# 0xC0000054/avif-format

Hardware: AMD Instinct MI355X
Metric: Mpixels/s + achieved HBM GB/s, 8K 32bpc→10-bit Rec.2100 PQ, 1 GPU (higher is better)
Workload: dtype f32

## Files before the change

avif-format_amd/csrc/device_math.h:

```cpp
#pragma once
#include <hip/hip_runtime.h>
#include <stdint.h>

namespace avifgpu {

#define AG_DEV __device__ __forceinline__

AG_DEV float nat_log2(float x) { return __builtin_amdgcn_logf(x); }
AG_DEV float nat_exp2(float x) { return __builtin_amdgcn_exp2f(x); }
AG_DEV float nat_rcp(float x)  { return __builtin_amdgcn_rcpf(x); }
AG_DEV float nat_sqrt(float x) { return __builtin_amdgcn_sqrtf(x); }

AG_DEV float max0(float v) { return __int_as_float(max(__float_as_int(v), 0)); }

AG_DEV float fast_pow(float x, float e) { return nat_exp2(e * nat_log2(x)); }

AG_DEV float fast_rcp_nr(float d)
{
    const float r = nat_rcp(d);
    return __builtin_fmaf(__builtin_fmaf(-d, r, 1.0f), r, r);
}

constexpr float kPqM1 = 2610.0f / 16384.0f;
constexpr float kPqM2 = 2523.0f / 4096.0f * 128.0f;
// ... 32 lines not shown
    const f32x2 l = { nat_log2(value.x), nat_log2(value.y) };
#endif
    const f32x2 e1 = __builtin_elementwise_fma((f32x2)kPqM1, l, (f32x2)log2_mult_m1);
    const f32x2 x = { nat_exp2(e1.x), nat_exp2(e1.y) };
    const f32x2 n = kPqC1 + kPqC2 * x;
    const f32x2 d = 1.0f + kPqC3 * x;
    const f32x2 r = { nat_rcp(d.x), nat_rcp(d.y) };
    const f32x2 q0 = n * r;
    const f32x2 q = __builtin_elementwise_fma(__builtin_elementwise_fma(-q0, d, n), r, q0);
    const f32x2 e2 = kPqM2 * f32x2{ nat_log2(q.x), nat_log2(q.y) };
    return f32x2{ nat_exp2_sat(e2.x), nat_exp2_sat(e2.y) };
}
AG_DEV float fast_linear_to_pq(float value, float mult)
{
    return fast_linear_to_pq01(value, kPqM1 * nat_log2(mult));
}

#ifndef AG_PQ_TAB_FORM
#define AG_PQ_TAB_FORM 2
#endif
#ifndef AG_PQ_ND_FMA
#define AG_PQ_ND_FMA 0
#endif
constexpr int kPqTabEntries = 512;
constexpr int kPqTabPad = 4;
constexpr int kPqTabCount = AG_PQ_TAB_FORM == 3 ? 3 : 2;
struct PqExpTable { float t[kPqTabCount][kPqTabEntries + kPqTabPad]; };
constexpr int kPqTabFloats = kPqTabCount * (kPqTabEntries + kPqTabPad);
constexpr float pq_pow2(int n) { float v = 1.0f; for (int i = 0; i < (n < 0 ? -n : n); ++i) v = n < 0 ? v * 0.5f : v * 2.0f; return v; }
constexpr PqExpTable make_pq_exp_table()
{
    PqExpTable t{};
    for (int i = 0; i < kPqTabEntries; ++i) {
        const int eb = i & 255;
        float F = 0.0f;
        int N = -100;
        if (i < 256 && eb != 0 && eb != 255) {
            const long long num = 2610LL * (eb - 126);
            long long n = (num + 8192) >> 14;
            if (((num + 8192) & 16383) == 0 && (n & 1)) n -= 1;
            F = (float)(num - n * 16384) / 16384.0f;
            N = (int)n;
        }
        if (AG_PQ_TAB_FORM == 3) { t.t[0][i] = F; t.t[1][i] = kPqC2 * pq_pow2(N); t.t[kPqTabCount - 1][i] = kPqC3 * pq_pow2(N); }
        else if (AG_PQ_TAB_FORM == 2) { t.t[0][i] = F; t.t[1][i] = pq_pow2(N); }
        else { constexpr int W = kPqTabEntries + kPqTabPad; t.t[(2 * i) / W][(2 * i) % W] = F; t.t[(2 * i + 1) / W][(2 * i + 1) % W] = pq_pow2(N); }
    }
    return t;
}
__device__ __attribute__((aligned(16))) const PqExpTable kPqExpTableConst = make_pq_exp_table();
static_assert(sizeof(PqExpTable) == kPqTabFloats * sizeof(float) && kPqTabFloats % 4 == 0, "copied as float4");
AG_DEV float* pq_exp_table()
{
    __shared__ __attribute__((aligned(16))) float tab[kPqTabFloats];
    return tab;
}
AG_DEV void pq_exp_table_fill(int tid, int nthreads)
{
    typedef float f4 __attribute__((ext_vector_type(4)));
    f4* dst = reinterpret_cast<f4*>(pq_exp_table());
    const f4* src = reinterpret_cast<const f4*>(&kPqExpTableConst);
    for (int i = tid; i < kPqTabFloats / 4; i += nthreads) dst[i] = src[i];
}
template <int NTHREADS> struct PqTableFill {
    typedef float f4 __attribute__((ext_vector_type(4)));
    static constexpr int kVec = kPqTabFloats / 4, N = (kVec + NTHREADS - 1) / NTHREADS;
    f4 v[N];
    AG_DEV void load(int tid)
    {
        const f4* src = reinterpret_cast<const f4*>(&kPqExpTableConst);
#pragma unroll
        for (int i = 0; i < N; ++i) { const int idx = tid + i * NTHREADS; v[i] = src[idx < kVec ? idx : kVec - 1]; }
        __builtin_amdgcn_sched_barrier(0);
    }
    AG_DEV void store(int tid)
    {
        f4* dst = reinterpret_cast<f4*>(pq_exp_table());
#pragma unroll
        for (int i = 0; i < N; ++i) { const int idx = tid + i * NTHREADS; dst[idx < kVec ? idx : kVec - 1] = v[i]; }
    }
};
AG_DEV void pq_table_barrier()
{
    __builtin_amdgcn_fence(__ATOMIC_RELEASE, "workgroup", "local");
    __builtin_amdgcn_s_barrier();
    __builtin_amdgcn_fence(__ATOMIC_ACQUIRE, "workgroup", "local");
}
AG_DEV uint32_t pq_tab_offset(float t) { return (__float_as_uint(t) >> (AG_PQ_TAB_FORM == 1 ? 20 : 21)) & (AG_PQ_TAB_FORM == 1 ? 0xff8u : 0x7fcu); }
AG_DEV float pq_tab_at(const float* tab, int which, uint32_t off)
{
    if (AG_PQ_TAB_FORM == 1) return *reinterpret_cast<const float*>(reinterpret_cast<const uint8_t*>(tab + which) + off);
    return *reinterpret_cast<const float*>(reinterpret_cast<const uint8_t*>(tab + which * (kPqTabEntries + kPqTabPad)) + off);
}
AG_DEV float pq_mantissa(float t) { return __uint_as_float((__float_as_uint(t) & 0x007fffffu) | 0x3f000000u); }
AG_DEV float fast_linear_to_pq01_hi(float value, float mult)
{
    const float* tab = pq_exp_table();
    const float t = value * mult;
    const uint32_t off = pq_tab_offset(t);
    const float y = nat_exp2(__builtin_fmaf(kPqM1, nat_log2(pq_mantissa(t)), pq_tab_at(tab, 0, off)));
    float n, d;
    if (AG_PQ_TAB_FORM == 3 && AG_PQ_ND_FMA) { n = __builtin_fmaf(pq_tab_at(tab, 1, off), y, kPqC1); d = __builtin_fmaf(pq_tab_at(tab, 2, off), y, 1.0f); }
    else if (AG_PQ_TAB_FORM == 3) { n = kPqC1 + pq_tab_at(tab, 1, off) * y; d = 1.0f + pq_tab_at(tab, 2, off) * y; }
    else if (AG_PQ_ND_FMA) { const float x = y * pq_tab_at(tab, 1, off); n = __builtin_fmaf(kPqC2, x, kPqC1); d = __builtin_fmaf(kPqC3, x, 1.0f); }
    else { const float x = y * pq_tab_at(tab, 1, off); n = kPqC1 + kPqC2 * x; d = 1.0f + kPqC3 * x; }
    return nat_exp2_sat(kPqM2 * nat_log2(near_ieee_div(n, d)));
}
AG_DEV f32x2 fast_linear_to_pq01_2_hi(f32x2 value, float mult)
{
    const float* tab = pq_exp_table();
    const f32x2 t = value * mult;
    const uint32_t o0 = pq_tab_offset(t.x), o1 = pq_tab_offset(t.y);
    const f32x2 F = { pq_tab_at(tab, 0, o0), pq_tab_at(tab, 0, o1) };
    const f32x2 l = { nat_log2(pq_mantissa(t.x)), nat_log2(pq_mantissa(t.y)) };
    const f32x2 e1 = __builtin_elementwise_fma((f32x2)kPqM1, l, F);
    const f32x2 y = { nat_exp2(e1.x), nat_exp2(e1.y) };
    f32x2 n, d;
// ... 403 lines not shown
```

avif-format_amd/csrc/write_kernels.hip:

```cpp
#include <hip/hip_runtime.h>
#include <cstdio>
#include <cstdlib>
#include <cstring>
#include <type_traits>
#include "kernel_params.h"
#include "staging.h"
#include "device_math.h"
#include "satword_f32.h"
#include "icc_pipeline32.h"
#include "../../include/avifgpu.h"

#pragma clang fp contract(off)

namespace avifgpu {

#ifndef AG_WRITE_PART
#define AG_WRITE_PART 0
#endif
constexpr bool kHerePlain  = AG_WRITE_PART != 36 && AG_WRITE_PART != 38 && AG_WRITE_PART != 1;
constexpr bool kHereIcc6   = AG_WRITE_PART == 0 || AG_WRITE_PART == 36;
constexpr bool kHereIcc8   = AG_WRITE_PART == 0 || AG_WRITE_PART == 38;
hipError_t launch_planes_d8(const WriteParams& p, int planes, bool dst16, int output, int xs, int ys, hipStream_t st, char* label);
hipError_t launch_planes_d16(const WriteParams& p, int planes, bool dst16, int output, int xs, int ys, hipStream_t st, char* label);
hipError_t launch_planes_d32(const WriteParams& p, int planes, bool dst16, int output, int xs, int ys, hipStream_t st, char* label);
// ... 1069 lines not shown
                        constexpr int v1 = YS ? 1 : 0;
                        R = (R + qflt(0, i0 + i1o, 0) + qflt(v1, i0, 0) + qflt(v1, i0 + i1o, 0)) * 0.25f;
                        G = (G + qflt(0, i0 + i1o, 1) + qflt(v1, i0, 1) + qflt(v1, i0 + i1o, 1)) * 0.25f;
                        B = (B + qflt(0, i0 + i1o, 2) + qflt(v1, i0, 2) + qflt(v1, i0 + i1o, 2)) * 0.25f;
                    }
                }
                const float cb = R * p.mcb[0] + G * p.mcb[1] + B * p.mcb[2];
                const float cr = R * p.mcr[0] + G * p.mcr[1] + B * p.mcr[2];
                cbv[j] = clip_round(cb + p.half, p.maxv);
                crv[j] = clip_round(cr + p.half, p.maxv);
            }
            const int ncvalid = (nvalid + (1 << XS) - 1) >> XS;
            store_samples<DST16, NC, true, ALIGNED>(p.dst[1] + (long long)gy * p.dst_stride[1] + (long long)(x0 >> XS) * DSZ, cbv, ncvalid);
            store_samples<DST16, NC, true, ALIGNED>(p.dst[2] + (long long)gy * p.dst_stride[2] + (long long)(x0 >> XS) * DSZ, crv, ncvalid);
        }
    }
}

#ifndef AG_STREAM_BLOCK
#define AG_STREAM_BLOCK 128
#endif
constexpr int kStreamWaves = AG_STREAM_BLOCK / 64;
#ifndef AG_F32_REF_BLOCK
#define AG_F32_REF_BLOCK 256
#endif
constexpr int kF32RefWaves = AG_F32_REF_BLOCK / 64;

typedef float    f32x4 __attribute__((ext_vector_type(4)));
typedef uint32_t u32x4 __attribute__((ext_vector_type(4)));
typedef uint32_t u32x2 __attribute__((ext_vector_type(2)));

typedef int i32x4 __attribute__((__vector_size__(16)));
typedef int i32x2 __attribute__((__vector_size__(8)));
AG_DEV __amdgpu_buffer_rsrc_t span_rsrc(const void* base, uint32_t bytes)
{
    return __builtin_amdgcn_make_buffer_rsrc(const_cast<void*>(base), 0, (int)bytes, 0x00020000);
}
template <bool NT> AG_DEV f32x4 span_load16(__amdgpu_buffer_rsrc_t r, uint32_t voff, uint32_t soff)
{
    if constexpr (AG_MATH_ONLY) return mo_value<f32x4>();
    const i32x4 v = __builtin_amdgcn_raw_buffer_load_b128(r, (int)voff, (int)soff, NT ? 2 : 0);
    return __builtin_bit_cast(f32x4, v);
}
template <bool NT> AG_DEV void span_store16(__amdgpu_buffer_rsrc_t r, uint32_t voff, u32x4 v)
{
    if constexpr (AG_MATH_ONLY) mo_sink(v); else __builtin_amdgcn_raw_buffer_store_b128(__builtin_bit_cast(i32x4, v), r, (int)voff, 0, NT ? 2 : 0);
}
template <bool NT> AG_DEV void span_store8(__amdgpu_buffer_rsrc_t r, uint32_t voff, u32x2 v)
// ... 136 lines not shown
#define AG_RGBA_PRIO 0
#endif
#ifndef AG_REF_PRIO
#define AG_REF_PRIO 0
#endif
#ifndef AG_INT_PRIO
#define AG_INT_PRIO 1
#endif
#ifndef AG_PREMUL_PAIR
#define AG_PREMUL_PAIR 1
#endif
#ifndef AG_REF_BUFFER_STORES
#define AG_REF_BUFFER_STORES 0
#endif
#ifndef AG_RGB16_BUFFER
#define AG_RGB16_BUFFER 0
#endif
#ifndef AG_IREF_BUFFER
#define AG_IREF_BUFFER 1
#endif
#ifndef AG_HOT444_BLOCK
#define AG_HOT444_BLOCK AG_F32_STREAM_BLOCK
#endif
#ifndef AG_MEASURE
#define AG_MEASURE 0
#endif
#ifndef AG_HOT444_GLOBAL
#define AG_HOT444_GLOBAL 0
#endif
constexpr int kHot444Waves = AG_HOT444_BLOCK / 64;
template <int TRANSFER, int PXL, bool NT>
__global__ __launch_bounds__(AG_HOT444_BLOCK) AG_F32_SGPRS void write_rgb32_ycbcr444_hot(const WriteParams p)
{
    constexpr int WPB = kHot444Waves;
    constexpr int K = 3 * PXL / 4;
    constexpr int SPAN_PX = 64 * PXL;
    constexpr int SPAN_DW = AG_HOT_F32_STRIP ? SpanStrip<K>::kDwords : SPAN_PX * 3 / 2;
    constexpr int LDW = 3 * PXL / 2;
    __shared__ __attribute__((aligned(16))) uint32_t strip[WPB][SPAN_DW];
    constexpr bool LATE = AG_PQ_LATE_FILL && TRANSFER == kTransferPqHi && !AG_HOT_PREFETCH;
    constexpr bool PRIO = AG_HOT_PRIO && TRANSFER == kTransferPqHi;
    if constexpr (PRIO) __builtin_amdgcn_s_setprio(3);
    PqTableFill<AG_HOT444_BLOCK> tfill;
    if constexpr (LATE) tfill.load((int)threadIdx.x); else pq_prologue<TRANSFER>();

    const int wave = wave_in_block();
    const int lane = threadIdx.x & 63;
    uint32_t* my = strip[wave];

    const uint32_t spans_per_row = ((uint32_t)p.width + SPAN_PX - 1) / SPAN_PX;
    const uint32_t total = spans_per_row * (uint32_t)p.nrows;
    const uint32_t step = gridDim.x * WPB;
    const uint32_t voff = (uint32_t)lane * 16u;

    auto issue = [&](uint32_t s, f32x4 (&dst)[K]) {
        const uint32_t r = s / spans_per_row;
        const uint32_t sx = s - r * spans_per_row;
        const int span_px = s < total ? min(SPAN_PX, p.width - (int)sx * SPAN_PX) : 0;
        if constexpr (AG_HOT444_GLOBAL && !AG_HOT_PREFETCH) {
            if (span_px == SPAN_PX) {
                const f32x4* g = reinterpret_cast<const f32x4*>(p.src + (long long)r * p.src_row_bytes + (long long)sx * (SPAN_PX * 12)) + lane;
#pragma unroll
                for (int k = 0; k < K; ++k) dst[k] = stream_load<NT>(g + 64 * k);
                return;
            }
        }
        const __amdgpu_buffer_rsrc_t rs = span_rsrc(p.src + (long long)(s < total ? r : 0) * p.src_row_bytes + (long long)(s < total ? sx : 0) * (SPAN_PX * 12), (uint32_t)span_px * 12u);
#pragma unroll
        for (int k = 0; k < K; ++k) dst[k] = span_load_cached(k, K) ? span_load16<false>(rs, voff, 1024u * k) : span_load16<NT>(rs, voff, 1024u * k);
    };
    f32x4 nxt[AG_HOT_PREFETCH ? K : 1];
    if constexpr (AG_HOT_PREFETCH) issue(blockIdx.x * WPB + wave, nxt);
    f32x4 cur[K];
    if constexpr (!AG_HOT_PREFETCH) issue(blockIdx.x * WPB + wave, cur);
    if constexpr (PRIO) __builtin_amdgcn_s_setprio(0);
    if constexpr (LATE) {
        tfill.store((int)threadIdx.x);
        pq_table_barrier();
    }
    for (uint32_t sidx = blockIdx.x * WPB + wave; sidx < total; sidx += step) {
        const uint32_t r = sidx / spans_per_row;
        const uint32_t sx = sidx - r * spans_per_row;
        const int span_px = min(SPAN_PX, p.width - (int)sx * SPAN_PX);
        if constexpr (AG_HOT_PREFETCH) {
#pragma unroll
            for (int k = 0; k < K; ++k) cur[k] = nxt[k];
            issue(sidx + step, nxt);
            __builtin_amdgcn_sched_barrier(0);
        }

        float R[PXL], G[PXL], B[PXL];
        if constexpr (AG_HOT_F32_STRIP) {
#pragma unroll
            for (int k = 0; k < K; ++k) cur[k] = oetf_level4<TRANSFER>(p, cur[k]);
            float c[3 * PXL];
            span_transpose<K>(reinterpret_cast<f32x4*>(my), lane, cur, c);
#pragma unroll
            for (int i = 0; i < PXL; ++i) { R[i] = c[strip_at(i, 0)]; G[i] = c[strip_at(i, 1)]; B[i] = c[strip_at(i, 2)]; }
        } else {
#pragma unroll
            for (int k = 0; k < K; ++k) {
// ... 86 lines not shown
    const IccPowTableF powT = { pow_t };
    const int wave = wave_in_block();
    const int lane = threadIdx.x & 63;
    const uint32_t voff = (uint32_t)lane * 16u;
    f32x4* my = reinterpret_cast<f32x4*>(strip[wave]);
    const float m0 = p.icc_m_f[0], m1 = p.icc_m_f[1], m2 = p.icc_m_f[2], m3 = p.icc_m_f[3], m4 = p.icc_m_f[4], m5 = p.icc_m_f[5],
                m6 = p.icc_m_f[6], m7 = p.icc_m_f[7], m8 = p.icc_m_f[8];
    const uint32_t spans_per_row = ((uint32_t)p.width + SPAN_PX - 1) / SPAN_PX;
    const uint32_t total = spans_per_row * (uint32_t)p.nrows;
    const uint32_t step = gridDim.x * kF32Waves;
    f32x4 cur[K];
    auto issue = [&](uint32_t s) {
        const uint32_t r = s / spans_per_row;
        const uint32_t sx = s - r * spans_per_row;
        const int span_px = s < total ? min(SPAN_PX, p.width - (int)sx * SPAN_PX) : 0;
        const __amdgpu_buffer_rsrc_t rs = span_rsrc(p.src + (long long)(s < total ? r : 0) * p.src_row_bytes + (long long)(s < total ? sx : 0) * (SPAN_PX * 12), (uint32_t)span_px * 12u);
#pragma unroll
        for (int k = 0; k < K; ++k) cur[k] = span_load_cached(k, K) ? span_load16<false>(rs, voff, 1024u * k) : span_load16<true>(rs, voff, 1024u * k);
    };
    issue(blockIdx.x * kF32Waves + wave);
    if constexpr (AG_SUB_PRIO && !OUTREF) __builtin_amdgcn_s_setprio(0);
    if constexpr (LATE) {
        tfill.store((int)threadIdx.x);
        pq_table_barrier();
    }
    for (uint32_t sidx = blockIdx.x * kF32Waves + wave; sidx < total; sidx += step) {
        const uint32_t r = sidx / spans_per_row;
        const uint32_t sx = sidx - r * spans_per_row;
        const int span_px = min(SPAN_PX, p.width - (int)sx * SPAN_PX);
        if constexpr (ICCV == 2) {
            const IccSimple q = icc_simple_load(p);
#pragma unroll
            for (int k = 0; k < K; ++k) icc_trc_simple4(q, cur[k]);
        }
        float c[PXL * 3];
        span_transpose<K>(my, lane, cur, c);
        uint32_t yv[PXL], cbv[PXL], crv[PXL];
        uint32_t pk[OUTREF ? 12 : 1];
#pragma unroll
        for (int i = 0; i < PXL; i += 2) {
            float t[6], q[6];
#pragma unroll
            for (int h = 0; h < 2; ++h) {
                const float R0 = c[strip_at(i + h, 0)], G0 = c[strip_at(i + h, 1)], B0 = c[strip_at(i + h, 2)];
                t[3 * h] = __builtin_fmaf(B0, m2, __builtin_fmaf(G0, m1, R0 * m0));
                t[3 * h + 1] = __builtin_fmaf(B0, m5, __builtin_fmaf(G0, m4, R0 * m3));
                t[3 * h + 2] = __builtin_fmaf(B0, m8, __builtin_fmaf(G0, m7, R0 * m6));
// ... 68 lines not shown
    const uint32_t spans_per_row = ((uint32_t)p.width + SPAN_PX - 1) / SPAN_PX;
    const uint32_t groups = ((uint32_t)p.nrows + VR - 1) >> YS;
    const uint32_t total = spans_per_row * groups;
    const uint32_t step = gridDim.x * kF32Waves;
    f32x4 v[VR][K];
    auto issue = [&](uint32_t s) {
        const uint32_t gy = s / spans_per_row;
        const uint32_t sx = s - gy * spans_per_row;
        const int span_px = s < total ? min(SPAN_PX, p.width - (int)sx * SPAN_PX) : 0;
#pragma unroll
        for (int vr = 0; vr < VR; ++vr) {
            const int r = s < total ? min((int)(gy * VR) + vr, p.rows_to_end - 1) : 0;
            const __amdgpu_buffer_rsrc_t rs = span_rsrc(p.src + (long long)r * p.src_row_bytes + (long long)(s < total ? sx : 0) * (SPAN_PX * 12), (uint32_t)span_px * 12u);
#pragma unroll
            for (int k = 0; k < K; ++k) v[vr][k] = span_load_cached(k, K) ? span_load16<false>(rs, voff, 1024u * k) : span_load16<true>(rs, voff, 1024u * k);
        }
    };
    const uint32_t w0 = blockIdx.x * kF32Waves + wave;
    auto span_of = [&](uint32_t it) -> uint32_t { return w0 + it * step; };
    issue(span_of(0));
    if constexpr (AG_SUB_PRIO) __builtin_amdgcn_s_setprio(0);
    if constexpr (LATE) {
        tfill.store((int)threadIdx.x);
        pq_table_barrier();
    }
    for (uint32_t it = 0, sidx = span_of(0); sidx < total; sidx = span_of(++it)) {
        const uint32_t gy = sidx / spans_per_row;
        const uint32_t sx = sidx - gy * spans_per_row;
        const int span_px = min(SPAN_PX, p.width - (int)sx * SPAN_PX);
        const int nv = span_px - PXL * lane;
        float acc[4][3];
#pragma unroll
        for (int vr = 0; vr < VR; ++vr) {
            float c[PXL * 3];
            if constexpr (ICC1) {
                if constexpr (ICCV == 2) {
                    const IccSimple q = icc_simple_load(p);
#pragma unroll
                    for (int k = 0; k < K; ++k) icc_trc_simple4(q, v[vr][k]);
                }
            } else {
#pragma unroll
                for (int k = 0; k < K; ++k) v[vr][k] = oetf_level4<TRANSFER>(p, v[vr][k]);
            }
            span_transpose<K>(reinterpret_cast<f32x4*>(my), lane, v[vr], c);
            if constexpr (ICC1) {
#pragma unroll
// ... 133 lines not shown
    constexpr int PXL = AG_RGBA_HOT_PXL, SPAN_PX = 64 * PXL;
    __shared__ __attribute__((aligned(16))) uint32_t strip[kRgbaWaves][SpanStrip<PXL>::kDwords];
    const int wave = wave_in_block();
    const int lane = threadIdx.x & 63;
    f32x4* my = reinterpret_cast<f32x4*>(strip[wave]);
    const uint32_t voff = (uint32_t)lane * 16u;

    const uint32_t spans_per_row = ((uint32_t)p.width + SPAN_PX - 1) / SPAN_PX;
    const uint32_t total = spans_per_row * (uint32_t)p.nrows;
    const uint32_t step = gridDim.x * kRgbaWaves;
    f32x4 v[PXL];
    auto issue = [&](uint32_t s) {
        const uint32_t r = s / spans_per_row;
        const uint32_t sx = s - r * spans_per_row;
        const int span_px = s < total ? min(SPAN_PX, p.width - (int)sx * SPAN_PX) : 0;
        const __amdgpu_buffer_rsrc_t rs = span_rsrc(p.src + (long long)(s < total ? r : 0) * p.src_row_bytes + (long long)(s < total ? sx : 0) * (SPAN_PX * 16), (uint32_t)span_px * 16u);
#pragma unroll
        for (int k = 0; k < PXL; ++k) v[k] = span_load16<true>(rs, voff, 1024u * k);
    };
    issue(blockIdx.x * kRgbaWaves + wave);
    if constexpr (AG_RGBA_PRIO) __builtin_amdgcn_s_setprio(0);
    if constexpr (LATE) {
        tfill.store((int)threadIdx.x);
        pq_table_barrier();
    }
    for (uint32_t sidx = blockIdx.x * kRgbaWaves + wave; sidx < total; sidx += step) {
        const uint32_t r = sidx / spans_per_row;
        const uint32_t sx = sidx - r * spans_per_row;
        const int span_px = min(SPAN_PX, p.width - (int)sx * SPAN_PX);
        rgba_levels<TRANSFER, ICCV, PXL>(p, v);
        float c[4 * PXL];
        span_transpose<PXL>(my, lane, v, c);
        f32x4 px[PXL];
#pragma unroll
        for (int j = 0; j < PXL; ++j) px[j] = f32x4{ c[4 * j], c[4 * j + 1], c[4 * j + 2], c[4 * j + 3] };
        uint32_t yv[PXL], cbv[PXL], crv[PXL], av[PXL];
#pragma unroll
        for (int i = 0; i < PXL; ++i) {
            const float R = px[i].x, G = px[i].y, B = px[i].z;
            av[i] = (uint32_t)px[i].w;
            yv[i] = luma_code_nc(p, R, G, B);
            cbv[i] = clip_round(R * p.mcb[0] + G * p.mcb[1] + B * p.mcb[2] + p.half, p.maxv);
            crv[i] = clip_round(R * p.mcr[0] + G * p.mcr[1] + B * p.mcr[2] + p.half, p.maxv);
        }
        const uint32_t* planes_v[4] = { yv, cbv, crv, av };
        const int nv = span_px - PXL * lane;
        const uint32_t svo = (uint32_t)lane * (PXL * 2u);
// ... 33 lines not shown
    f32x4* my = reinterpret_cast<f32x4*>(strip[wave]);
    const uint32_t voff = (uint32_t)lane * 16u;
    const uint32_t spans_per_row = ((uint32_t)p.width + SPAN_PX - 1) / SPAN_PX;
    const uint32_t groups = ((uint32_t)p.nrows + VR - 1) >> YS;
    const uint32_t total = spans_per_row * groups;
    const uint32_t step = gridDim.x * kRgbaWaves;
    f32x4 v[VR][PXL];
    auto issue = [&](uint32_t s) {
        const uint32_t gy = s / spans_per_row;
        const uint32_t sx = s - gy * spans_per_row;
        const int span_px = s < total ? min(SPAN_PX, p.width - (int)sx * SPAN_PX) : 0;
#pragma unroll
        for (int vr = 0; vr < VR; ++vr) {
            const int r = s < total ? min((int)(gy * VR) + vr, p.rows_to_end - 1) : 0;
            const __amdgpu_buffer_rsrc_t rs = span_rsrc(p.src + (long long)r * p.src_row_bytes + (long long)(s < total ? sx : 0) * (SPAN_PX * 16), (uint32_t)span_px * 16u);
#pragma unroll
            for (int k = 0; k < PXL; ++k) v[vr][k] = span_load16<true>(rs, voff, 1024u * k);
        }
    };
    issue(blockIdx.x * kRgbaWaves + wave);
    if constexpr (AG_RGBA_PRIO) __builtin_amdgcn_s_setprio(0);
    if constexpr (LATE) {
        tfill.store((int)threadIdx.x);
        pq_table_barrier();
    }
    for (uint32_t sidx = blockIdx.x * kRgbaWaves + wave; sidx < total; sidx += step) {
        const uint32_t gy = sidx / spans_per_row;
        const uint32_t sx = sidx - gy * spans_per_row;
        const int span_px = min(SPAN_PX, p.width - (int)sx * SPAN_PX);
        const int nv = span_px - PXL * lane;
        float acc[2][3];
#pragma unroll
        for (int vr = 0; vr < VR; ++vr) {
            rgba_levels<TRANSFER, 0, PXL>(p, v[vr]);
            float c[4 * PXL];
            span_transpose<PXL>(my, lane, v[vr], c);
            const int r = (int)(gy * VR) + vr;
            if (r < p.nrows) {
                uint32_t yv[PXL], av[PXL];
#pragma unroll
                for (int i = 0; i < PXL; ++i) { yv[i] = luma_code_nc(p, c[4 * i], c[4 * i + 1], c[4 * i + 2]); av[i] = (uint32_t)c[4 * i + 3]; }
                const long long xo = (long long)sx * (SPAN_PX * 2);
                span_store_samples4<true>(p.dst[0] + (long long)r * p.dst_stride[0] + xo, (uint32_t)span_px, (uint32_t)lane, u32x2{ yv[0] | (yv[1] << 16), yv[2] | (yv[3] << 16) });
                span_store_samples4<true>(p.dst[3] + (long long)r * p.dst_stride[3] + xo, (uint32_t)span_px, (uint32_t)lane, u32x2{ av[0] | (av[1] << 16), av[2] | (av[3] << 16) });
            }
            if constexpr (!NEAREST) {
                if (span_px & 1) {
// ... 817 lines not shown
    if constexpr (AG_REF_PRIO) __builtin_amdgcn_s_setprio(3);
    PqTableFill<AG_F32_REF_BLOCK> tfill;
    if constexpr (LATE) tfill.load((int)threadIdx.x); else pq_prologue<TRANSFER>();
    constexpr int K = 4;
    const int lane = threadIdx.x & 63;
    const int wave = wave_in_block();
    const uint32_t n4 = (uint32_t)p.width * PLANES / 4;
    const uint32_t chunks = (n4 + 64 * K - 1) / (64 * K);
    const uint32_t total = chunks * (uint32_t)p.nrows;
    const uint32_t step = gridDim.x * kF32RefWaves;
    f32x4 v[K];
    auto issue = [&](uint32_t w) {
        const uint32_t r = w / chunks;
        const uint32_t c = w - r * chunks;
        const __amdgpu_buffer_rsrc_t rs = span_rsrc(p.src + (long long)(w < total ? r : 0) * p.src_row_bytes, w < total ? n4 * 16u : 0u);
        const uint32_t vo = (c * (64 * K) + (uint32_t)lane) * 16u;
#pragma unroll
        for (int k = 0; k < K; ++k) v[k] = span_load16<true>(rs, vo, 1024u * k);
    };
    issue(blockIdx.x * kF32RefWaves + wave);
    if constexpr (AG_REF_PRIO) __builtin_amdgcn_s_setprio(0);
    if constexpr (LATE) {
        tfill.store((int)threadIdx.x);
        pq_table_barrier();
    }
    for (uint32_t widx = blockIdx.x * kF32RefWaves + wave; widx < total; widx += step) {
        const uint32_t r = widx / chunks;
        const uint32_t c = widx - r * chunks;
        u32x2* dp = reinterpret_cast<u32x2*>(p.dst[0] + (long long)r * p.dst_stride[0]);
        uint32_t idx[K];
#pragma unroll
        for (int k = 0; k < K; ++k) idx[k] = c * (64 * K) + 64 * k + lane;
#pragma unroll
        for (int k = 0; k < K; k += 2) {
            float t[8];
            uint32_t q[8], ca[2] = { 0, 0 };
#pragma unroll
            for (int h = 0; h < 2; ++h) {
                float s0 = v[k + h].x, s1 = v[k + h].y, s2 = v[k + h].z, s3 = v[k + h].w;
                if constexpr (PLANES == 4) {
                    const float a = cxx_clamp(s3, 0.0f, 1.0f);
                    if (p.premultiply && a < 1.0f) {
                        s0 = (a == 0.0f) ? 0.0f : cxx_clamp(s0, 0.0f, 1.0f) * a;
                        s1 = (a == 0.0f) ? 0.0f : cxx_clamp(s1, 0.0f, 1.0f) * a;
                        s2 = (a == 0.0f) ? 0.0f : cxx_clamp(s2, 0.0f, 1.0f) * a;
                    }
                    ca[h] = (uint32_t)__builtin_amdgcn_fmed3f(a * p.maxf, 0.0f, p.maxf);
// ... 7 lines not shown
                const float tc[6] = { t[0], t[1], t[2], t[4], t[5], t[6] };
                uint32_t qc[6];
                oetf_codes<TRANSFER>(p, tc, qc);
                q[0] = qc[0]; q[1] = qc[1]; q[2] = qc[2]; q[3] = ca[0]; q[4] = qc[3]; q[5] = qc[4]; q[6] = qc[5]; q[7] = ca[1];
            } else {
                oetf_codes<TRANSFER>(p, t, q);
            }
#pragma unroll
            for (int h = 0; h < 2; ++h) {
                u32x2 o = { q[4 * h] | (q[4 * h + 1] << 16), q[4 * h + 2] | (q[4 * h + 3] << 16) };
                if constexpr (AG_REF_BUFFER_STORES) {
                    span_store8<true>(span_rsrc(dp, n4 * 8u), idx[k + h] * 8u, o);
                } else {
                    if (idx[k + h] >= n4) continue;
                    stream_store<true>(dp + idx[k + h], o);
                }
            }
        }
        if (widx + step < total) issue(widx + step);
    }
}

template <int DEPTH, int TRANSFER>
__global__ __launch_bounds__(AG_F32_REF_BLOCK) void write_ga_stream(const WriteParams p)
{
    static_assert(DEPTH == 16 || DEPTH == 32, "u16 or f32 samples");
    constexpr bool LATE = AG_PQ_LATE_FILL && DEPTH == 32 && TRANSFER == kTransferPqHi;
    PqTableFill<AG_F32_REF_BLOCK> tfill;
    if constexpr (LATE) tfill.load((int)threadIdx.x); else if constexpr (DEPTH == 32) pq_prologue<TRANSFER>();
    constexpr int K = 4;
    constexpr int PXV = DEPTH == 16 ? 4 : 2;
    const int lane = threadIdx.x & 63;
    const int wave = wave_in_block();
    const uint32_t nv = (uint32_t)p.width / PXV;
    const uint32_t chunks = (nv + 64 * K - 1) / (64 * K);
    const uint32_t total = chunks * (uint32_t)p.nrows;
    const uint32_t step = gridDim.x * kF32RefWaves;
    f32x4 v[K];
    auto issue = [&](uint32_t w) {
        const uint32_t r = w / chunks;
        const uint32_t c = w - r * chunks;
        const __amdgpu_buffer_rsrc_t rs = span_rsrc(p.src + (long long)(w < total ? r : 0) * p.src_row_bytes, w < total ? nv * 16u : 0u);
        const uint32_t vo = (c * (64 * K) + (uint32_t)lane) * 16u;
#pragma unroll
        for (int k = 0; k < K; ++k) v[k] = span_load16<true>(rs, vo, 1024u * k);
    };
    issue(blockIdx.x * kF32RefWaves + wave);
    if constexpr (LATE) {
        tfill.store((int)threadIdx.x);
        pq_table_barrier();
    }
    for (uint32_t widx = blockIdx.x * kF32RefWaves + wave; widx < total; widx += step) {
        const uint32_t r = widx / chunks;
        const uint32_t c = widx - r * chunks;
        const uint32_t row_bytes = (uint32_t)p.width * 2u;
        const __amdgpu_buffer_rsrc_t ry = span_rsrc(p.dst[0] + (long long)r * p.dst_stride[0], row_bytes);
        const __amdgpu_buffer_rsrc_t ra = span_rsrc(p.dst[3] + (long long)r * p.dst_stride[3], row_bytes);
#pragma unroll
        for (int k = 0; k < K; ++k) {
            const uint32_t idx = c * (64 * K) + 64 * k + (uint32_t)lane;
            const u32x4 in = __builtin_bit_cast(u32x4, v[k]);
            const uint32_t w4[4] = { in.x, in.y, in.z, in.w };
            uint32_t yq[PXV], aq[PXV];
#pragma unroll
            for (int i = 0; i < PXV; ++i) {
                uint32_t sm[2], q[4];
                if constexpr (DEPTH == 16) { sm[0] = w4[i] & 0xffffu; sm[1] = w4[i] >> 16; }
                else { sm[0] = w4[2 * i]; sm[1] = w4[2 * i + 1]; }
                stage_a<DEPTH, 2, TRANSFER>(p, sm, q);
                yq[i] = q[0]; aq[i] = q[3];
            }
            if constexpr (DEPTH == 16) {
                span_store8<true>(ry, idx * 8u, u32x2{ yq[0] | (yq[1] << 16), yq[2] | (yq[3] << 16) });
                span_store8<true>(ra, idx * 8u, u32x2{ aq[0] | (aq[1] << 16), aq[2] | (aq[3] << 16) });
            } else {
// ... 421 lines not shown
        ((long long)p.width * planes * (depth / 8)) % 16 == 0 && (p.src_row_bytes & 15) == 0 && (reinterpret_cast<uintptr_t>(p.src) & 15) == 0 &&
        ((reinterpret_cast<uintptr_t>(p.dst[0]) | (uintptr_t)p.dst_stride[0]) & 15) == 0) {
        const long long nv = (long long)p.width * planes * (depth / 8) / 16;
        const long long waves = ((nv + 255) / 256) * p.nrows;
        if (waves == 0) return hipSuccess;
        if (waves + 8LL * 65536 * 4 < 0x7fffffffLL) {
            const long long need = (waves + kStreamWaves - 1) / kStreamWaves;
            const long long blocks = capped_blocks(need, AG_STREAM_BLOCK_CAP * 4 / kStreamWaves, variant);
            snprintf(label, kLabelBytes, "write_int_ref_stream<depth=%d,planes=%d,dst16=%d>", depth, planes, (int)dst16);
            label_cap(label, blocks, need, AG_STREAM_BLOCK_CAP * 4 / kStreamWaves);
#define AG_IREF(D, P) do { if (dst16) hipLaunchKernelGGL((write_int_ref_stream<D, P, true>), dim3((int)blocks), dim3(AG_STREAM_BLOCK), 0, st, p); \
                           else hipLaunchKernelGGL((write_int_ref_stream<D, P, false>), dim3((int)blocks), dim3(AG_STREAM_BLOCK), 0, st, p); } while (0)
            if (depth == 8) AG_IREF(8, 4);
            else { if (planes == 4) AG_IREF(16, 4); else if (planes == 1) AG_IREF(16, 1); else AG_IREF(16, 3); }
#undef AG_IREF
            return hipGetLastError();
        }
    }
    if (depth == 16 && (p.width % 4) == 0 && (variant & 1) && planes == 2 && dst16 && p.dst[3] != nullptr && (p.src_row_bytes & 3) == 0 && (reinterpret_cast<uintptr_t>(p.src) & 3) == 0 &&
        ((reinterpret_cast<uintptr_t>(p.dst[0]) | reinterpret_cast<uintptr_t>(p.dst[3]) | (uintptr_t)p.dst_stride[0] | (uintptr_t)p.dst_stride[3]) & 3) == 0) {
        const long long waves = (((long long)p.width / 4 + 255) / 256) * p.nrows;
        if (waves == 0) return hipSuccess;
        if (waves + 8LL * 65536 * 4 < 0x7fffffffLL) {
            const long long need = (waves + kF32RefWaves - 1) / kF32RefWaves;
            const long long blocks = capped_blocks(need, AG_STREAM_BLOCK_CAP * 4 / kF32RefWaves, variant);
            snprintf(label, kLabelBytes, "write_ga_stream<depth=16>");
            label_cap(label, blocks, need, AG_STREAM_BLOCK_CAP * 4 / kF32RefWaves);
            hipLaunchKernelGGL((write_ga_stream<16, AVIFGPU_TRANSFER_CLIP>), dim3((int)blocks), dim3(AG_F32_REF_BLOCK), 0, st, p);
            return hipGetLastError();
        }
    }
    if (AG_RGB8_HOT && (variant & 1) && p.icc8_s1 == nullptr && depth == 8 && planes == 3 && !dst16 && output == AVIFGPU_OUT_YCBCR && p.maxv == 255 &&
        (p.width % 8) == 0 && (p.src_row_bytes & 3) == 0 && (reinterpret_cast<uintptr_t>(p.src) & 3) == 0 &&
        ((reinterpret_cast<uintptr_t>(p.dst[0]) | reinterpret_cast<uintptr_t>(p.dst[1]) | reinterpret_cast<uintptr_t>(p.dst[2]) |
          (uintptr_t)p.dst_stride[0] | (uintptr_t)p.dst_stride[1] | (uintptr_t)p.dst_stride[2]) & 3) == 0) {
        const long long spans = (long long)((p.width + 1023) / 1024) * ((p.nrows + (1 << ys) - 1) >> ys);
        if (spans == 0) return hipSuccess;
        if (spans + 8LL * 65536 * 4 < 0x7fffffffLL) {
            const int wpb = ys ? 2 : 4;
            const long long need = (spans + wpb - 1) / wpb;
            const long long blocks = capped_blocks(need, AG_STREAM_BLOCK_CAP * 4 / wpb, variant);
            snprintf(label, kLabelBytes, "write_rgb8_ycbcr_hot<xs=%d,ys=%d,nearest=%d>", xs, ys, (xs || ys) ? p.nearest : 0);
            label_cap(label, blocks, need, AG_STREAM_BLOCK_CAP * 4 / wpb);
#define AG_R8(XS_, YS_, NR_) hipLaunchKernelGGL((write_rgb8_ycbcr_hot<XS_, YS_, NR_, (YS_ ? 2 : 4)>), dim3((int)blocks), dim3(64 * (YS_ ? 2 : 4)), 0, st, p)
            if (xs == 0) AG_R8(0, 0, false);
            else if (ys == 0) { if (p.nearest) AG_R8(1, 0, true); else AG_R8(1, 0, false); }
            else { if (p.nearest) AG_R8(1, 1, true); else AG_R8(1, 1, false); }
#undef AG_R8
            return hipGetLastError();
        }
    }
// ... 108 lines not shown
            const long long blocks = capped_blocks(need, AG_STREAM_BLOCK_CAP * 4 / kStreamWaves, variant);
            snprintf(label, kLabelBytes, "write_rgb16_ycbcr_sub_hot<ys=%d%s>", ys, dst16 ? "" : ",to8");
            label_cap(label, blocks, need, AG_STREAM_BLOCK_CAP * 4 / kStreamWaves);
            if (dst16) { if (ys) hipLaunchKernelGGL((write_rgb16_ycbcr_sub_hot<1>), dim3((int)blocks), dim3(AG_STREAM_BLOCK), 0, st, p);
                         else hipLaunchKernelGGL((write_rgb16_ycbcr_sub_hot<0>), dim3((int)blocks), dim3(AG_STREAM_BLOCK), 0, st, p); }
            else { if (ys) hipLaunchKernelGGL((write_rgb16_ycbcr_sub_hot<1, true>), dim3((int)blocks), dim3(AG_STREAM_BLOCK), 0, st, p);
                   else hipLaunchKernelGGL((write_rgb16_ycbcr_sub_hot<0, true>), dim3((int)blocks), dim3(AG_STREAM_BLOCK), 0, st, p); }
            return hipGetLastError();
        }
    }
    *taken = false;
    return hipSuccess;
}
#endif
#if AG_WRITE_PART == 0 || AG_WRITE_PART == 3
hipError_t launch_stream_f32_sub_rgba(const WriteParams& p, int depth, int planes, bool dst16, int output, int xs, int ys, int variant, hipStream_t st, char* label, bool* taken)
{
    *taken = true;
    if (depth == 32 && (p.width % 2) == 0 && (variant & 1) && planes == 2 && dst16 && p.dst[3] != nullptr && (p.src_row_bytes & 3) == 0 && (reinterpret_cast<uintptr_t>(p.src) & 3) == 0 &&
        ((reinterpret_cast<uintptr_t>(p.dst[0]) | reinterpret_cast<uintptr_t>(p.dst[3]) | (uintptr_t)p.dst_stride[0] | (uintptr_t)p.dst_stride[3]) & 3) == 0) {
        const long long waves = (((long long)p.width / 2 + 255) / 256) * p.nrows;
        if (waves == 0) return hipSuccess;
        if (waves + 8LL * 65536 * 4 < 0x7fffffffLL) {
            const long long need = (waves + kF32RefWaves - 1) / kF32RefWaves;
            const long long blocks = capped_blocks(need, AG_STREAM_BLOCK_CAP * 4 / kF32RefWaves, variant);
            snprintf(label, kLabelBytes, "write_ga_stream<depth=32,transfer=%d>", p.transfer);
            label_cap(label, blocks, need, AG_STREAM_BLOCK_CAP * 4 / kF32RefWaves);
            if (p.transfer == AVIFGPU_TRANSFER_PQ) {
                if (pq_hi_launch(p)) hipLaunchKernelGGL((write_ga_stream<32, kTransferPqHi>), dim3((int)blocks), dim3(AG_F32_REF_BLOCK), 0, st, p);
                else hipLaunchKernelGGL((write_ga_stream<32, AVIFGPU_TRANSFER_PQ>), dim3((int)blocks), dim3(AG_F32_REF_BLOCK), 0, st, p);
            } else {
                hipLaunchKernelGGL((write_ga_stream<32, AVIFGPU_TRANSFER_CLIP>), dim3((int)blocks), dim3(AG_F32_REF_BLOCK), 0, st, p);
            }
            return hipGetLastError();
        }
    }
    if ((variant & 1) && p.icc_trc_type[0] == 0 && p.icc_s_tab == nullptr && depth == 32 && planes == 4 && dst16 && output == AVIFGPU_OUT_YCBCR && xs == 1 &&
        (p.src_row_bytes & 3) == 0 && (reinterpret_cast<uintptr_t>(p.src) & 3) == 0 && p.dst[3] != nullptr &&
        ((reinterpret_cast<uintptr_t>(p.dst[0]) | reinterpret_cast<uintptr_t>(p.dst[1]) | reinterpret_cast<uintptr_t>(p.dst[2]) |
          reinterpret_cast<uintptr_t>(p.dst[3]) | (uintptr_t)p.dst_stride[0] | (uintptr_t)p.dst_stride[1] | (uintptr_t)p.dst_stride[2] |
          (uintptr_t)p.dst_stride[3]) & 3) == 0) {
        const long long spans = (long long)((p.width + 255) / 256) * ((p.nrows + (1 << ys) - 1) >> ys);
        if (spans == 0) return hipSuccess;
        if (spans + 8LL * 65536 * 4 < 0x7fffffffLL) {
            const long long need = (spans + kRgbaWaves - 1) / kRgbaWaves;
            const long long blocks = capped_blocks(need, AG_RGBA_BLOCK_CAP * 4 / kRgbaWaves, variant);
            snprintf(label, kLabelBytes, "write_rgba32_ycbcra_sub_hot<transfer=%d,xs=1,ys=%d,nearest=%d>", p.transfer, ys, p.nearest);
            label_cap(label, blocks, need, AG_RGBA_BLOCK_CAP * 4 / kRgbaWaves);
#define AG_RSUB3(TR, YS_, NR_) hipLaunchKernelGGL((write_rgba32_ycbcra_sub_hot<TR, YS_, NR_>), dim3((int)blocks), dim3(AG_RGBA_STREAM_BLOCK), 0, st, p)
#define AG_RSUB2(TR, YS_) do { if (p.nearest) AG_RSUB3(TR, YS_, true); else AG_RSUB3(TR, YS_, false); } while (0)
#define AG_RSUB(TR) do { if (ys) AG_RSUB2(TR, 1); else AG_RSUB2(TR, 0); } while (0)
            switch (p.transfer) {
            case AVIFGPU_TRANSFER_PQ:       if (pq_hi_launch(p)) AG_RSUB(kTransferPqHi); else AG_RSUB(AVIFGPU_TRANSFER_PQ); break;
            case AVIFGPU_TRANSFER_HLG:      AG_RSUB(AVIFGPU_TRANSFER_HLG); break;
            case AVIFGPU_TRANSFER_SMPTE428: AG_RSUB(AVIFGPU_TRANSFER_SMPTE428); break;
// ... 452 lines not shown
            if (icc4) { hipLaunchKernelGGL((write_rgb32_icc1_ycbcr444_hot<AVIFGPU_TRANSFER_CLIP, 4>), dim3((int)blocks), dim3(AG_F32_STREAM_BLOCK), 0, st, p); return hipGetLastError(); }
#define AG_I444(TR) do { if (icc2) hipLaunchKernelGGL((write_rgb32_icc1_ycbcr444_hot<TR, 2>), dim3((int)blocks), dim3(AG_F32_STREAM_BLOCK), 0, st, p); \
                         else hipLaunchKernelGGL((write_rgb32_icc1_ycbcr444_hot<TR, 1>), dim3((int)blocks), dim3(AG_F32_STREAM_BLOCK), 0, st, p); } while (0)
            switch (p.transfer) {
            case AVIFGPU_TRANSFER_PQ:       if (pq_hi_launch(p)) AG_I444(kTransferPqHi); else AG_I444(AVIFGPU_TRANSFER_PQ); break;
            case AVIFGPU_TRANSFER_HLG:      AG_I444(AVIFGPU_TRANSFER_HLG); break;
            case AVIFGPU_TRANSFER_SMPTE428: AG_I444(AVIFGPU_TRANSFER_SMPTE428); break;
            default:                        AG_I444(AVIFGPU_TRANSFER_CLIP); break;
            }
#undef AG_I444
            return hipGetLastError();
        }
    }
    if ((variant & 1) && p.icc_trc_type[0] == 0 && depth == 32 && planes == 3 && dst16 && output == AVIFGPU_OUT_YCBCR && xs == 0 && ys == 0 &&
        (p.src_row_bytes & 3) == 0 && (reinterpret_cast<uintptr_t>(p.src) & 3) == 0 &&
        ((reinterpret_cast<uintptr_t>(p.dst[0]) | reinterpret_cast<uintptr_t>(p.dst[1]) | reinterpret_cast<uintptr_t>(p.dst[2]) |
          (uintptr_t)p.dst_stride[0] | (uintptr_t)p.dst_stride[1] | (uintptr_t)p.dst_stride[2]) & 3) == 0) {
        {
            const bool px8 = variant & 2, nt = variant & 4;
            const int span_px = px8 ? 512 : 256;
            const long long spans = (long long)((p.width + span_px - 1) / span_px) * p.nrows;
            if (spans == 0) return hipSuccess;
            if (spans + 8LL * 65536 * 4 < 0x7fffffffLL) {
            constexpr int WPB = kHot444Waves;
            const long long need = (spans + WPB - 1) / WPB;
            const long long cap = 256LL * 512 * 4 / WPB;
            const long long blocks = capped_blocks(need, cap, variant);
            snprintf(label, kLabelBytes, "write_rgb32_ycbcr444_hot<transfer=%d,pxl=%d,nt=%d>", p.transfer, px8 ? 8 : 4, (int)nt);
            label_cap(label, blocks, need, cap);
#if AG_MEASURE
            static const size_t lds_pad = [] { const char* e = getenv("AVIFGPU_DEBUG_LDS_PAD"); const long v = e ? atol(e) : 0; return (size_t)(v < 0 ? 0 : (v > 140000 ? 140000 : v)); }();
#else
            constexpr size_t lds_pad = 0;
#endif
#define AG_HOT3(TR, PX, NT_) hipLaunchKernelGGL((write_rgb32_ycbcr444_hot<TR, PX, NT_>), dim3((int)blocks), dim3(AG_HOT444_BLOCK), lds_pad, st, p)
#define AG_HOT2(TR, PX) do { if (nt) AG_HOT3(TR, PX, true); else AG_HOT3(TR, PX, false); } while (0)
#define AG_HOT1(TR) do { if (px8) AG_HOT2(TR, 8); else AG_HOT2(TR, 4); } while (0)
            switch (p.transfer) {
            case AVIFGPU_TRANSFER_PQ:       if (pq_hi_launch(p)) AG_HOT1(kTransferPqHi); else AG_HOT1(AVIFGPU_TRANSFER_PQ); break;
            case AVIFGPU_TRANSFER_HLG:      AG_HOT1(AVIFGPU_TRANSFER_HLG); break;
            case AVIFGPU_TRANSFER_SMPTE428: AG_HOT1(AVIFGPU_TRANSFER_SMPTE428); break;
            default:                        AG_HOT1(AVIFGPU_TRANSFER_CLIP); break;
            }
            return hipGetLastError();
            }
        }
    }
    switch (depth) {
    case 8:  return launch_planes_d8(p, planes, dst16, output, xs, ys, st, label);
    case 16: return launch_planes_d16(p, planes, dst16, output, xs, ys, st, label);
    default: return launch_planes_d32(p, planes, dst16, output, xs, ys, st, label);
    }
}
#endif

}
```

Measured before the change: 336,800.

## Halve PQ LDS table and use smaller blocks for line-aligned hot 444 path

Shrinks the PQ exponent lookup table from 512 to 256 entries by folding the sign bit into the mantissa term instead of the index, so each block fills less LDS. Adds a block-size template parameter to the hot 444 kernel and launches 128-thread blocks when buffers and strides are 128-byte aligned. It also uses a wave barrier when a block is a single wave, and defaults the f32 reference kernel to 64 threads. Smaller blocks and tables are meant to cut the per-block table-fill and barrier cost and improve scheduling, at the cost of more blocks and more template instantiations.

```diff
diff --git a/avif-format_amd/csrc/device_math.h b/avif-format_amd/csrc/device_math.h
--- a/avif-format_amd/csrc/device_math.h
+++ b/avif-format_amd/csrc/device_math.h
@@ -78,20 +78,22 @@
 #ifndef AG_PQ_ND_FMA
 #define AG_PQ_ND_FMA 0
 #endif
-constexpr int kPqTabEntries = 512;
+constexpr int kPqTabEntries = 256;
 constexpr int kPqTabPad = 4;
 constexpr int kPqTabCount = AG_PQ_TAB_FORM == 3 ? 3 : 2;
-struct PqExpTable { float t[kPqTabCount][kPqTabEntries + kPqTabPad]; };
-constexpr int kPqTabFloats = kPqTabCount * (kPqTabEntries + kPqTabPad);
+constexpr int kPqTabGap = AG_PQ_TAB_FORM == 1 ? 0 : kPqTabPad;
+struct PqExpTable { float t[kPqTabCount][kPqTabEntries]; };
+constexpr int kPqTabConstFloats = kPqTabCount * kPqTabEntries;
+constexpr int kPqTabFloats = kPqTabCount * kPqTabEntries + (kPqTabCount - 1) * kPqTabGap;
 constexpr float pq_pow2(int n) { float v = 1.0f; for (int i = 0; i < (n < 0 ? -n : n); ++i) v = n < 0 ? v * 0.5f : v * 2.0f; return v; }
 constexpr PqExpTable make_pq_exp_table()
 {
     PqExpTable t{};
     for (int i = 0; i < kPqTabEntries; ++i) {
-        const int eb = i & 255;
+        const int eb = i;
         float F = 0.0f;
         int N = -100;
-        if (i < 256 && eb != 0 && eb != 255) {
+        if (eb != 0 && eb != 255) {
             const long long num = 2610LL * (eb - 126);
             long long n = (num + 8192) >> 14;
             if (((num + 8192) & 16383) == 0 && (n & 1)) n -= 1;
@@ -100,12 +102,14 @@
         }
         if (AG_PQ_TAB_FORM == 3) { t.t[0][i] = F; t.t[1][i] = kPqC2 * pq_pow2(N); t.t[kPqTabCount - 1][i] = kPqC3 * pq_pow2(N); }
         else if (AG_PQ_TAB_FORM == 2) { t.t[0][i] = F; t.t[1][i] = pq_pow2(N); }
-        else { constexpr int W = kPqTabEntries + kPqTabPad; t.t[(2 * i) / W][(2 * i) % W] = F; t.t[(2 * i + 1) / W][(2 * i + 1) % W] = pq_pow2(N); }
+        else { constexpr int W = kPqTabEntries; t.t[(2 * i) / W][(2 * i) % W] = F; t.t[(2 * i + 1) / W][(2 * i + 1) % W] = pq_pow2(N); }
     }
     return t;
 }
 __device__ __attribute__((aligned(16))) const PqExpTable kPqExpTableConst = make_pq_exp_table();
-static_assert(sizeof(PqExpTable) == kPqTabFloats * sizeof(float) && kPqTabFloats % 4 == 0, "copied as float4");
+static_assert(sizeof(PqExpTable) == kPqTabConstFloats * sizeof(float) && kPqTabEntries % 4 == 0 && kPqTabGap % 4 == 0, "copied as float4");
+constexpr int kPqTabVec = kPqTabConstFloats / 4;
+AG_DEV int pq_tab_lds_vec(int i) { return i + (i / (kPqTabEntries / 4)) * (kPqTabGap / 4); }
 AG_DEV float* pq_exp_table()
 {
     __shared__ __attribute__((aligned(16))) float tab[kPqTabFloats];
@@ -116,11 +120,11 @@
     typedef float f4 __attribute__((ext_vector_type(4)));
     f4* dst = reinterpret_cast<f4*>(pq_exp_table());
     const f4* src = reinterpret_cast<const f4*>(&kPqExpTableConst);
-    for (int i = tid; i < kPqTabFloats / 4; i += nthreads) dst[i] = src[i];
+    for (int i = tid; i < kPqTabVec; i += nthreads) dst[pq_tab_lds_vec(i)] = src[i];
 }
 template <int NTHREADS> struct PqTableFill {
     typedef float f4 __attribute__((ext_vector_type(4)));
-    static constexpr int kVec = kPqTabFloats / 4, N = (kVec + NTHREADS - 1) / NTHREADS;
+    static constexpr int kVec = kPqTabVec, N = (kVec + NTHREADS - 1) / NTHREADS;
     f4 v[N];
     AG_DEV void load(int tid)
     {
@@ -133,22 +137,24 @@
     {
         f4* dst = reinterpret_cast<f4*>(pq_exp_table());
 #pragma unroll
-        for (int i = 0; i < N; ++i) { const int idx = tid + i * NTHREADS; dst[idx < kVec ? idx : kVec - 1] = v[i]; }
+        for (int i = 0; i < N; ++i) { const int idx = tid + i * NTHREADS; dst[pq_tab_lds_vec(idx < kVec ? idx : kVec - 1)] = v[i]; }
     }
 };
+template <int NTHREADS>
 AG_DEV void pq_table_barrier()
 {
     __builtin_amdgcn_fence(__ATOMIC_RELEASE, "workgroup", "local");
-    __builtin_amdgcn_s_barrier();
+    if constexpr (NTHREADS > 64) __builtin_amdgcn_s_barrier(); else __builtin_amdgcn_wave_barrier();
     __builtin_amdgcn_fence(__ATOMIC_ACQUIRE, "workgroup", "local");
 }
-AG_DEV uint32_t pq_tab_offset(float t) { return (__float_as_uint(t) >> (AG_PQ_TAB_FORM == 1 ? 20 : 21)) & (AG_PQ_TAB_FORM == 1 ? 0xff8u : 0x7fcu); }
+AG_DEV uint32_t pq_tab_offset(float t) { return (__float_as_uint(t) >> (AG_PQ_TAB_FORM == 1 ? 20 : 21)) & (AG_PQ_TAB_FORM == 1 ? 0x7f8u : 0x3fcu); }
+static_assert((0x3fcu >> 2) == kPqTabEntries - 1 && (0x7f8u >> 3) == kPqTabEntries - 1, "the index is the exponent field alone: no form reads past its table");
 AG_DEV float pq_tab_at(const float* tab, int which, uint32_t off)
 {
     if (AG_PQ_TAB_FORM == 1) return *reinterpret_cast<const float*>(reinterpret_cast<const uint8_t*>(tab + which) + off);
-    return *reinterpret_cast<const float*>(reinterpret_cast<const uint8_t*>(tab + which * (kPqTabEntries + kPqTabPad)) + off);
-}
-AG_DEV float pq_mantissa(float t) { return __uint_as_float((__float_as_uint(t) & 0x007fffffu) | 0x3f000000u); }
+    return *reinterpret_cast<const float*>(reinterpret_cast<const uint8_t*>(tab + which * (kPqTabEntries + kPqTabGap)) + off);
+}
+AG_DEV float pq_mantissa(float t) { return __uint_as_float((__float_as_uint(t) & 0x807fffffu) | 0x3f000000u); }
 AG_DEV float fast_linear_to_pq01_hi(float value, float mult)
 {
     const float* tab = pq_exp_table();
diff --git a/avif-format_amd/csrc/write_kernels.hip b/avif-format_amd/csrc/write_kernels.hip
--- a/avif-format_amd/csrc/write_kernels.hip
+++ b/avif-format_amd/csrc/write_kernels.hip
@@ -1115,8 +1115,12 @@
 #endif
 constexpr int kStreamWaves = AG_STREAM_BLOCK / 64;
 #ifndef AG_F32_REF_BLOCK
-#define AG_F32_REF_BLOCK 256
-#endif
+#define AG_F32_REF_BLOCK 64
+#endif
+#ifndef AG_GA_BLOCK
+#define AG_GA_BLOCK 256
+#endif
+constexpr int kGaWaves = AG_GA_BLOCK / 64;
 constexpr int kF32RefWaves = AG_F32_REF_BLOCK / 64;
 
 typedef float    f32x4 __attribute__((ext_vector_type(4)));
@@ -1299,17 +1303,20 @@
 #ifndef AG_HOT444_BLOCK
 #define AG_HOT444_BLOCK AG_F32_STREAM_BLOCK
 #endif
+#ifndef AG_HOT444_BLOCK_LINES
+#define AG_HOT444_BLOCK_LINES 128
+#endif
 #ifndef AG_MEASURE
 #define AG_MEASURE 0
 #endif
 #ifndef AG_HOT444_GLOBAL
 #define AG_HOT444_GLOBAL 0
 #endif
-constexpr int kHot444Waves = AG_HOT444_BLOCK / 64;
-template <int TRANSFER, int PXL, bool NT>
-__global__ __launch_bounds__(AG_HOT444_BLOCK) AG_F32_SGPRS void write_rgb32_ycbcr444_hot(const WriteParams p)
-{
-    constexpr int WPB = kHot444Waves;
+static_assert(AG_HOT444_BLOCK % 64 == 0 && AG_HOT444_BLOCK_LINES % 64 == 0, "whole waves");
+template <int TRANSFER, int PXL, bool NT, int BLOCK>
+__global__ __launch_bounds__(BLOCK) AG_F32_SGPRS void write_rgb32_ycbcr444_hot(const WriteParams p)
+{
+    constexpr int WPB = BLOCK / 64;
     constexpr int K = 3 * PXL / 4;
     constexpr int SPAN_PX = 64 * PXL;
     constexpr int SPAN_DW = AG_HOT_F32_STRIP ? SpanStrip<K>::kDwords : SPAN_PX * 3 / 2;
@@ -1318,7 +1325,7 @@
     constexpr bool LATE = AG_PQ_LATE_FILL && TRANSFER == kTransferPqHi && !AG_HOT_PREFETCH;
     constexpr bool PRIO = AG_HOT_PRIO && TRANSFER == kTransferPqHi;
     if constexpr (PRIO) __builtin_amdgcn_s_setprio(3);
-    PqTableFill<AG_HOT444_BLOCK> tfill;
+    PqTableFill<BLOCK> tfill;
     if constexpr (LATE) tfill.load((int)threadIdx.x); else pq_prologue<TRANSFER>();
 
     const int wave = wave_in_block();
@@ -1353,7 +1360,7 @@
     if constexpr (PRIO) __builtin_amdgcn_s_setprio(0);
     if constexpr (LATE) {
         tfill.store((int)threadIdx.x);
-        pq_table_barrier();
+        pq_table_barrier<BLOCK>();
     }
     for (uint32_t sidx = blockIdx.x * WPB + wave; sidx < total; sidx += step) {
         const uint32_t r = sidx / spans_per_row;
@@ -1486,7 +1493,7 @@
     if constexpr (AG_SUB_PRIO && !OUTREF) __builtin_amdgcn_s_setprio(0);
     if constexpr (LATE) {
         tfill.store((int)threadIdx.x);
-        pq_table_barrier();
+        pq_table_barrier<AG_F32_STREAM_BLOCK>();
     }
     for (uint32_t sidx = blockIdx.x * kF32Waves + wave; sidx < total; sidx += step) {
         const uint32_t r = sidx / spans_per_row;
@@ -1601,7 +1608,7 @@
     if constexpr (AG_SUB_PRIO) __builtin_amdgcn_s_setprio(0);
     if constexpr (LATE) {
         tfill.store((int)threadIdx.x);
-        pq_table_barrier();
+        pq_table_barrier<AG_F32_STREAM_BLOCK>();
     }
     for (uint32_t it = 0, sidx = span_of(0); sidx < total; sidx = span_of(++it)) {
         const uint32_t gy = sidx / spans_per_row;
@@ -1781,7 +1788,7 @@
     if constexpr (AG_RGBA_PRIO) __builtin_amdgcn_s_setprio(0);
     if constexpr (LATE) {
         tfill.store((int)threadIdx.x);
-        pq_table_barrier();
+        pq_table_barrier<AG_RGBA_STREAM_BLOCK>();
     }
     for (uint32_t sidx = blockIdx.x * kRgbaWaves + wave; sidx < total; sidx += step) {
         const uint32_t r = sidx / spans_per_row;
@@ -1861,7 +1868,7 @@
     if constexpr (AG_RGBA_PRIO) __builtin_amdgcn_s_setprio(0);
     if constexpr (LATE) {
         tfill.store((int)threadIdx.x);
-        pq_table_barrier();
+        pq_table_barrier<AG_RGBA_STREAM_BLOCK>();
     }
     for (uint32_t sidx = blockIdx.x * kRgbaWaves + wave; sidx < total; sidx += step) {
         const uint32_t gy = sidx / spans_per_row;
@@ -2725,7 +2732,7 @@
     if constexpr (AG_REF_PRIO) __builtin_amdgcn_s_setprio(0);
     if constexpr (LATE) {
         tfill.store((int)threadIdx.x);
-        pq_table_barrier();
+        pq_table_barrier<AG_F32_REF_BLOCK>();
     }
     for (uint32_t widx = blockIdx.x * kF32RefWaves + wave; widx < total; widx += step) {
         const uint32_t r = widx / chunks;
@@ -2779,11 +2786,11 @@
 }
 
 template <int DEPTH, int TRANSFER>
-__global__ __launch_bounds__(AG_F32_REF_BLOCK) void write_ga_stream(const WriteParams p)
+__global__ __launch_bounds__(AG_GA_BLOCK) void write_ga_stream(const WriteParams p)
 {
     static_assert(DEPTH == 16 || DEPTH == 32, "u16 or f32 samples");
     constexpr bool LATE = AG_PQ_LATE_FILL && DEPTH == 32 && TRANSFER == kTransferPqHi;
-    PqTableFill<AG_F32_REF_BLOCK> tfill;
+    PqTableFill<AG_GA_BLOCK> tfill;
     if constexpr (LATE) tfill.load((int)threadIdx.x); else if constexpr (DEPTH == 32) pq_prologue<TRANSFER>();
     constexpr int K = 4;
     constexpr int PXV = DEPTH == 16 ? 4 : 2;
@@ -2792,7 +2799,7 @@
     const uint32_t nv = (uint32_t)p.width / PXV;
     const uint32_t chunks = (nv + 64 * K - 1) / (64 * K);
     const uint32_t total = chunks * (uint32_t)p.nrows;
-    const uint32_t step = gridDim.x * kF32RefWaves;
+    const uint32_t step = gridDim.x * kGaWaves;
     f32x4 v[K];
     auto issue = [&](uint32_t w) {
         const uint32_t r = w / chunks;
@@ -2802,12 +2809,12 @@
 #pragma unroll
         for (int k = 0; k < K; ++k) v[k] = span_load16<true>(rs, vo, 1024u * k);
     };
-    issue(blockIdx.x * kF32RefWaves + wave);
+    issue(blockIdx.x * kGaWaves + wave);
     if constexpr (LATE) {
         tfill.store((int)threadIdx.x);
-        pq_table_barrier();
-    }
-    for (uint32_t widx = blockIdx.x * kF32RefWaves + wave; widx < total; widx += step) {
+        pq_table_barrier<AG_GA_BLOCK>();
+    }
+    for (uint32_t widx = blockIdx.x * kGaWaves + wave; widx < total; widx += step) {
         const uint32_t r = widx / chunks;
         const uint32_t c = widx - r * chunks;
         const uint32_t row_bytes = (uint32_t)p.width * 2u;
@@ -3275,11 +3282,11 @@
         const long long waves = (((long long)p.width / 4 + 255) / 256) * p.nrows;
         if (waves == 0) return hipSuccess;
         if (waves + 8LL * 65536 * 4 < 0x7fffffffLL) {
-            const long long need = (waves + kF32RefWaves - 1) / kF32RefWaves;
-            const long long blocks = capped_blocks(need, AG_STREAM_BLOCK_CAP * 4 / kF32RefWaves, variant);
+            const long long need = (waves + kGaWaves - 1) / kGaWaves;
+            const long long blocks = capped_blocks(need, AG_STREAM_BLOCK_CAP * 4 / kGaWaves, variant);
             snprintf(label, kLabelBytes, "write_ga_stream<depth=16>");
-            label_cap(label, blocks, need, AG_STREAM_BLOCK_CAP * 4 / kF32RefWaves);
-            hipLaunchKernelGGL((write_ga_stream<16, AVIFGPU_TRANSFER_CLIP>), dim3((int)blocks), dim3(AG_F32_REF_BLOCK), 0, st, p);
+            label_cap(label, blocks, need, AG_STREAM_BLOCK_CAP * 4 / kGaWaves);
+            hipLaunchKernelGGL((write_ga_stream<16, AVIFGPU_TRANSFER_CLIP>), dim3((int)blocks), dim3(AG_GA_BLOCK), 0, st, p);
             return hipGetLastError();
         }
     }
@@ -3434,15 +3441,15 @@
         const long long waves = (((long long)p.width / 2 + 255) / 256) * p.nrows;
         if (waves == 0) return hipSuccess;
         if (waves + 8LL * 65536 * 4 < 0x7fffffffLL) {
-            const long long need = (waves + kF32RefWaves - 1) / kF32RefWaves;
-            const long long blocks = capped_blocks(need, AG_STREAM_BLOCK_CAP * 4 / kF32RefWaves, variant);
+            const long long need = (waves + kGaWaves - 1) / kGaWaves;
+            const long long blocks = capped_blocks(need, AG_STREAM_BLOCK_CAP * 4 / kGaWaves, variant);
             snprintf(label, kLabelBytes, "write_ga_stream<depth=32,transfer=%d>", p.transfer);
-            label_cap(label, blocks, need, AG_STREAM_BLOCK_CAP * 4 / kF32RefWaves);
+            label_cap(label, blocks, need, AG_STREAM_BLOCK_CAP * 4 / kGaWaves);
             if (p.transfer == AVIFGPU_TRANSFER_PQ) {
-                if (pq_hi_launch(p)) hipLaunchKernelGGL((write_ga_stream<32, kTransferPqHi>), dim3((int)blocks), dim3(AG_F32_REF_BLOCK), 0, st, p);
-                else hipLaunchKernelGGL((write_ga_stream<32, AVIFGPU_TRANSFER_PQ>), dim3((int)blocks), dim3(AG_F32_REF_BLOCK), 0, st, p);
+                if (pq_hi_launch(p)) hipLaunchKernelGGL((write_ga_stream<32, kTransferPqHi>), dim3((int)blocks), dim3(AG_GA_BLOCK), 0, st, p);
+                else hipLaunchKernelGGL((write_ga_stream<32, AVIFGPU_TRANSFER_PQ>), dim3((int)blocks), dim3(AG_GA_BLOCK), 0, st, p);
             } else {
-                hipLaunchKernelGGL((write_ga_stream<32, AVIFGPU_TRANSFER_CLIP>), dim3((int)blocks), dim3(AG_F32_REF_BLOCK), 0, st, p);
+                hipLaunchKernelGGL((write_ga_stream<32, AVIFGPU_TRANSFER_CLIP>), dim3((int)blocks), dim3(AG_GA_BLOCK), 0, st, p);
             }
             return hipGetLastError();
         }
@@ -3941,7 +3948,10 @@
             const long long spans = (long long)((p.width + span_px - 1) / span_px) * p.nrows;
             if (spans == 0) return hipSuccess;
             if (spans + 8LL * 65536 * 4 < 0x7fffffffLL) {
-            constexpr int WPB = kHot444Waves;
+            const uintptr_t bases = reinterpret_cast<uintptr_t>(p.src) | reinterpret_cast<uintptr_t>(p.dst[0]) | reinterpret_cast<uintptr_t>(p.dst[1]) | reinterpret_cast<uintptr_t>(p.dst[2]);
+            const uintptr_t strides = (uintptr_t)p.src_row_bytes | (uintptr_t)p.dst_stride[0] | (uintptr_t)p.dst_stride[1] | (uintptr_t)p.dst_stride[2];
+            const bool lines = (bases & 127) == 0 && (p.nrows == 1 || (strides & 127) == 0);
+            const int WPB = (lines ? AG_HOT444_BLOCK_LINES : AG_HOT444_BLOCK) / 64;
             const long long need = (spans + WPB - 1) / WPB;
             const long long cap = 256LL * 512 * 4 / WPB;
             const long long blocks = capped_blocks(need, cap, variant);
@@ -3952,7 +3962,8 @@
 #else
             constexpr size_t lds_pad = 0;
 #endif
-#define AG_HOT3(TR, PX, NT_) hipLaunchKernelGGL((write_rgb32_ycbcr444_hot<TR, PX, NT_>), dim3((int)blocks), dim3(AG_HOT444_BLOCK), lds_pad, st, p)
+#define AG_HOT3(TR, PX, NT_) do { if (lines) hipLaunchKernelGGL((write_rgb32_ycbcr444_hot<TR, PX, NT_, AG_HOT444_BLOCK_LINES>), dim3((int)blocks), dim3(AG_HOT444_BLOCK_LINES), lds_pad, st, p); \
+                                  else hipLaunchKernelGGL((write_rgb32_ycbcr444_hot<TR, PX, NT_, AG_HOT444_BLOCK>), dim3((int)blocks), dim3(AG_HOT444_BLOCK), lds_pad, st, p); } while (0)
 #define AG_HOT2(TR, PX) do { if (nt) AG_HOT3(TR, PX, true); else AG_HOT3(TR, PX, false); } while (0)
 #define AG_HOT1(TR) do { if (px8) AG_HOT2(TR, 8); else AG_HOT2(TR, 4); } while (0)
             switch (p.transfer) {
```

After: 341,500, median of 6. 1.4% higher.
